# HumaticsLAB/SEAM-Match-RCNN

Measured on AMD Instinct MI355X. Metric: video-clips/sec (10f x 800^2, 32 ROI/f, 1k gallery), higher is better.
Workload: dtype f32; 1 GPU; configs[1] full pipeline, fixed ROIs: 10 frames 800x800 -> ResNet-50-FPN + RPN head -> RoIAlign 14x14 (32 ROI/frame) -> mask head -> match trunk x2 -> SEAM NLB + attention pool (32 seq x 10) -> pair logits vs 1000-product bank -> top-20; hip_graph=False, hip_streams=2, frames=10, rois_per_frame=32, gallery=1000, topk=20, parallelism=single GPU

## Files before the change

include/seam_hip.h:

```cpp
#ifndef SEAM_HIP_H
#define SEAM_HIP_H

#include <stdint.h>

#ifdef __cplusplus
extern "C" {
#endif

typedef void* seam_stream_t;

int seam_version(void);
int seam_fastdiv_exact(unsigned d, unsigned long long n_max);
const char* seam_error_string(int code);

int seam_option_count(void);
const char* seam_option_name(int index);
int seam_set_option(const char* name, int value);
int seam_get_option(const char* name, int* value);

int seam_conv_kred(int C, int R, int S);
int seam_conv_rows_padded(int K);
int seam_conv_tile(int M, int K);
int seam_conv_tile_prec(int prec, int M, int K);
int seam_conv_tile_taps(int prec, int M, int K, int taps);
// ... 185 lines not shown

int seam_paste_masks_f32(const float* masks, const float* boxes, float* out, int K, int H, int W,
                         seam_stream_t stream);

int seam_mask_select_f32(const float* logits, const int64_t* labels, float* prob, int K, int ncls,
                         seam_stream_t stream);

int seam_mask_select_f16(const void* logits, const int64_t* labels, float* prob, int K, int ncls,
                         seam_stream_t stream);

int seam_pack_conv_weight_bx3(const float* w, void* w_packed, float* tmp, int K, int Cin, int R, int S,
                              int Cstore, int mode, seam_stream_t stream);
int seam_conv2d_bx3(const float* x, const void* w_packed, const float* scale, const float* shift,
                    const float* residual, float* y, int N, int H, int W, int C, int K, int R, int S,
                    int stride, int pad, int relu, seam_stream_t stream);

int seam_wino_supported(int C, int K, int R, int S, int stride);
long long seam_wino_weight_floats(int K, int Cstore);
int seam_wino_slot_fill_pct(int N, int H, int W, int C, int K, int pad);
int seam_wino_tile_variant(int N, int H, int W, int C, int K, int pad);
int seam_pack_conv_weight_wino_f32(const float* w, float* u_packed, int K, int Cin, int Cstore, int mode,
                                   seam_stream_t stream);
int seam_conv3x3_wino_f32(const float* x, const float* u_packed, const float* scale, const float* shift,
                          const float* residual, float* y, int N, int H, int W, int C, int K, int pad, int relu,
                          seam_stream_t stream);

int seam_linear_narrow_supported(int C, int K);
int seam_pack_linear_narrow_f32(const float* w, float* w_packed, int K, int C, seam_stream_t stream);
int seam_linear_narrow_f32(const float* x, const float* w_packed, const float* bias, float* y, long long M, int C, int K,
                           int relu, seam_stream_t stream);
// ... 117 lines not shown
```

seam-match-rcnn_amd/_native.py:

```python
from __future__ import annotations

import ctypes as C
import os

import torch

_HERE = os.path.dirname(os.path.abspath(__file__))
LIB_PATH = os.environ.get("SEAM_LIB_PATH") or os.path.join(_HERE, "lib", "libseam_hip.so")

_p = C.c_void_p
_i = C.c_int
_f = C.c_float
_i64 = C.c_int64

class TrunkLayer(C.Structure):
    _fields_ = [("w", C.c_void_p), ("u", C.c_void_p), ("u24", C.c_void_p), ("scale", C.c_void_p), ("shift", C.c_void_p)]


SIGNATURES = {
    "seam_version": (_i, []),
    "seam_fastdiv_exact": (_i, [C.c_uint, C.c_ulonglong]),
    "seam_error_string": (C.c_char_p, [_i]),
    "seam_option_count": (_i, []),
    "seam_option_name": (C.c_char_p, [_i]),
# ... 20 lines not shown
    "seam_pack_conv1x1_pc_f32": (_i, [_p, _p, _i, _i, _p]),
    "seam_conv1x1_pc_f32": (_i, [_p, _p, _p, _p, _p, _p, C.c_longlong, _i, _i, _i, _p]),
    "seam_conv1x1_sw_config": (_i, [_i, _i, _i, _i]),
    "seam_conv1x1_sw_f32": (_i, [_p, _p, _p, _p, _p, _p, _i, _i, _i, _i, _i, _i, _i, _i, _i, _i, _p]),
    "seam_conv1x1_swh_config": (_i, [C.c_longlong, _i, _i, _i]),
    "seam_conv1x1_f16pc_supported": (_i, [C.c_longlong, _i, _i]),
    "seam_conv1x1_f16pc_weight_halves": (C.c_longlong, [_i, _i]),
    "seam_pack_conv1x1_weight_f16pc": (_i, [_p, _p, _i, _i, _p]),
    "seam_conv1x1_f16pc": (_i, [_p, _p, _p, _p, _p, _p, C.c_longlong, _i, _i, _i, _p]),
    "seam_conv1x1_swh_f16": (_i, [_p, _p, _p, _p, _p, _p, _p, C.c_longlong, _i, _i, _i, _i, _i, _i, _i, _i, _i, _p]),
    "seam_stem_s2d_swh_f16": (_i, [_p, _p, _p, _p, _p, _i, _i, _i, _i, _p]),
    "seam_conv2d_dual_f16": (_i, [_p, _p, _p, _p, _p, _p, _i, _i, _i, _i, _i, _i, _i, _i, _i, _i, _p]),
    "seam_conv2d_upres_f32": (_i, [_p, _p, _p, _p, _p, _p, _i, _i, _i, _i, _i, _i, _i, _i, _i, _i, _i, _i, _p]),
    "seam_pack_conv_weight_bx3": (_i, [_p, _p, _p, _i, _i, _i, _i, _i, _i, _p]),
    "seam_conv2d_bx3": (_i, [_p, _p, _p, _p, _p, _p, _i, _i, _i, _i, _i, _i, _i, _i, _i, _i, _p]),
    "seam_wino_supported": (_i, [_i, _i, _i, _i, _i]),
    "seam_wino_weight_floats": (C.c_longlong, [_i, _i]),
    "seam_wino_slot_fill_pct": (_i, [_i, _i, _i, _i, _i, _i]),
    "seam_wino_tile_variant": (_i, [_i, _i, _i, _i, _i, _i]),
    "seam_pack_conv_weight_wino_f32": (_i, [_p, _p, _i, _i, _i, _i, _p]),
    "seam_wino_issue_slots": (C.c_longlong, [_i, _i, _i, _i, _i, _i]),
    "seam_wino24_issue_slots": (C.c_longlong, [_i, _i, _i, _i, _i, _i]),
    "seam_wino24_variant": (_i, [_i, _i, _i, _i, _i, _i]),
    "seam_wino24_form": (_i, [_i, _i, _i, _i, _i, _i]),
    "seam_wino24_weight_floats": (C.c_longlong, [_i, _i]),
    "seam_pack_conv_weight_wino24_f32": (_i, [_p, _p, _i, _i, _i, _i, _p]),
    "seam_conv3x3_wino24_f32": (_i, [_p, _p, _p, _p, _p, _p, _i, _i, _i, _i, _i, _i, _i, _p]),
    "seam_conv3x3_wino_f32": (_i, [_p, _p, _p, _p, _p, _p, _i, _i, _i, _i, _i, _i, _i, _p]),
    "seam_conv3x3_f16pc_supported": (_i, [_i, _i, _i, _i, _i, _i]),
    "seam_conv3x3_f16pc_pays": (_i, [_i, _i, _i, _i, _i, _i]),
# ... 153 lines not shown
```

seam-match-rcnn_amd/csrc/seam_conv.hip:

```cpp
#include <hip/hip_runtime.h>
#include <stdint.h>
#include <stdio.h>
#include <stdlib.h>
#include "seam_fastdiv.h"
#include "seam_fpn_common.h"
#include "seam_opts.h"

typedef float f32x4 __attribute__((ext_vector_type(4)));
typedef float f32x16 __attribute__((ext_vector_type(16)));
typedef _Float16 f16x8 __attribute__((ext_vector_type(8)));
typedef unsigned u32x4 __attribute__((ext_vector_type(4)));

namespace {

constexpr int CHUNK_BYTES = 128;
constexpr int LDB = CHUNK_BYTES + 16;
constexpr unsigned kOob = 0x80000000u;

struct ConvArgs {
    const void* x;
    const void* w;
    const float* scale;
    const float* shift;
    const void* res;
// ... 716 lines not shown
#pragma unroll
                for (int r = 0; r < 16; ++r)
                    rv[r] = __builtin_bit_cast(float, __builtin_amdgcn_raw_buffer_load_b32(r_rsrc, nok ? eo[r] * 4u : kOob, 0, 0));
            }
#pragma unroll
            for (int r = 0; r < 16; ++r) {
                float v = acc[i][j][r] * sc + sh;
                if (p.res) v = p.relu == 2 ? (rv[r] > 0.f ? v : 0.f) : v + rv[r];
                if (p.relu == 1) v = fmaxf(v, 0.f);
                __builtin_amdgcn_raw_buffer_store_b32(__builtin_bit_cast(unsigned, v), y_rsrc, nok ? eo[r] * 4u : kOob, 0, 0);
            }
        }
    }
}

__global__ void split_weight_kernel(const float* __restrict__ in, unsigned short* __restrict__ out, size_t total) {
    for (size_t i = (size_t)blockIdx.x * blockDim.x + threadIdx.x; i < total; i += (size_t)gridDim.x * blockDim.x) {
        const float x = in[i];
        const __bf16 h = (__bf16)x;
        const __bf16 l = (__bf16)(x - (float)h);
        const size_t rowchunk = i >> 5;
        const int col = (int)(i & 31);
        out[rowchunk * 64 + col] = __builtin_bit_cast(unsigned short, h);
        out[rowchunk * 64 + 32 + col] = __builtin_bit_cast(unsigned short, l);
    }
}

template <typename T>
__global__ void pack_weight_kernel(const float* __restrict__ w, T* __restrict__ out, int K, int Cin, int R, int S,
                                   int Cstore, int kred, int rows, int bn, int mode) {
// ... 46 lines not shown

template <typename T>
int pack_weight(const float* w, void* w_packed, int K, int Cin, int R, int S, int Cstore, int mode, void* stream) {
    constexpr int BKE = CHUNK_BYTES / (int)sizeof(T), EPV = 16 / (int)sizeof(T);
    if ((Cstore % EPV) || (Cstore >= BKE && Cstore % BKE)) return (int)hipErrorInvalidValue;
    const int kred = kred_of<T>(Cstore, R, S);
    const int rows = ((K + 63) / 64) * 64;
    const size_t total = (size_t)rows * kred;
    int grid = (int)((total + 255) / 256);
    if (grid > 4096) grid = 4096;
    hipLaunchKernelGGL(pack_weight_kernel<T>, dim3(grid), dim3(256), 0, (hipStream_t)stream, w, (T*)w_packed, K, Cin, R, S,
                       Cstore, kred, rows, rows % 128 == 0 ? 128 : 64, mode);
    return (int)hipGetLastError();
}

enum Prec { P_F32 = 0, P_F16 = 1, P_BX3 = 2 };

inline int tile_weight(int prec, int bm, int bn, int taps) {
    const int area = bm * bn;
    if (prec == P_F32) return area == 256 * 128 ? 100 : area == 128 * 128 ? 100 : area == 64 * 64 ? 125 : 110;
    if (prec == P_F16 && area == 256 * 128) return taps >= 9 ? 92 : 105;
    return area == 256 * 128 ? 95 : area == 128 * 128 ? 100 : area == 64 * 64 ? 200 : 150;
}

inline void choose_tile(int prec, int M, int K, int& best_bm, int& best_bn, int taps = 1) {
    const int rows = ((K + 63) / 64) * 64;
    const int slab = rows % 128 == 0 ? 128 : 64;
    const int force = seam_opt::get(seam_opt::CONV_TILE);
    if (force) {
        const int fm = force / 1000, fn = force % 1000;
        if ((fm == 256 || fm == 128 || fm == 64) && (fn == 128 || fn == 64) &&
            fn <= slab && (fm != 256 || fn == 128)) {
            best_bm = fm; best_bn = fn;
            return;
        }
    }
    long best_cost = -1;
    best_bm = 128;
    best_bn = slab;
    for (int bm = 256; bm >= 64; bm >>= 1)
        for (int bn = slab; bn >= 64; bn -= 64) {
            if (bm == 256 && (bn != 128 || prec == P_F32)) continue;
            const long nb = (long)((M + bm - 1) / bm) * (rows / bn);
            const long cost = ((nb + 255) / 256) * bm * bn * tile_weight(prec, bm, bn, taps);
            if (best_cost < 0 || cost < best_cost) { best_cost = cost; best_bm = bm; best_bn = bn; }
        }
}

struct DualSrc { const void* x2; int H2, W2, C2, stride2; };

inline void set_row_split(ConvArgs& a) {
    const unsigned long long howo = (unsigned long long)a.Ho * a.Wo;
    a.m_HoWo = seam_fastdiv::magic(howo);
    a.m_Wo = seam_fastdiv::magic((unsigned long long)a.Wo);
    a.div_fast = (a.Ho > 0 && a.Wo > 0 && (howo >= 256 || seam_fastdiv::exact(howo, howo + 256)) &&
                  seam_fastdiv::exact((unsigned long long)a.Wo, howo)) ? 1 : 0;
}
// ... 59 lines not shown
            else if (best_bm == 128) hipLaunchKernelGGL((conv_igemm<T, 128, 64, 4, true>), grid, dim3(256), dyn, st, a);
            else if (best_bn == 128) hipLaunchKernelGGL((conv_igemm<T, 64, 128, 4, true>), grid, dim3(256), dyn, st, a);
            else hipLaunchKernelGGL((conv_igemm<T, 64, 64, 4, true>), grid, dim3(256), dyn, st, a);
            return (int)hipGetLastError();
        }
    }
    if (best_bm == 256) hipLaunchKernelGGL((conv_igemm<T, 256, 128, 8>), grid, dim3(512), dyn, st, a);
    else if (best_bm == 128 && best_bn == 128) hipLaunchKernelGGL((conv_igemm<T, 128, 128, 4>), grid, dim3(256), dyn, st, a);
    else if (best_bm == 128) hipLaunchKernelGGL((conv_igemm<T, 128, 64, 4>), grid, dim3(256), dyn, st, a);
    else if (best_bn == 128) hipLaunchKernelGGL((conv_igemm<T, 64, 128, 4>), grid, dim3(256), dyn, st, a);
    else hipLaunchKernelGGL((conv_igemm<T, 64, 64, 4>), grid, dim3(256), dyn, st, a);
    return (int)hipGetLastError();
}

int conv2d_bx3(const void* x, const void* w_packed, const float* scale, const float* shift, const void* residual, void* y,
               int N, int H, int W, int C, int K, int R, int S, int stride, int pad, int relu, void* stream) {
    if ((C % 4) || (C >= 32 && C % 32) || N <= 0 || K <= 0) return (int)hipErrorInvalidValue;
    ConvArgs a;
    a.x = x; a.w = w_packed; a.scale = scale; a.shift = shift; a.res = residual; a.y = y;
    a.N = N; a.H = H; a.W = W; a.C = C;
    a.Ho = (H + 2 * pad - R) / stride + 1;
    a.Wo = (W + 2 * pad - S) / stride + 1;
    a.K = K; a.R = R; a.S = S; a.stride = stride; a.pad = pad;
    a.kred = kred_of<float>(C, R, S);
    a.M = N * a.Ho * a.Wo;
    a.relu = relu;
    a.y_f32 = 1;
    a.vec_epi = 0;
    a.epi_prio = 0;
    a.rH = 0; a.rW = 0;
    a.x2 = nullptr; a.H2 = a.W2 = a.C2 = a.stride2 = 0;
    set_row_split(a);
    if (a.Ho <= 0 || a.Wo <= 0) return (int)hipErrorInvalidValue;
    const int rows = ((K + 63) / 64) * 64;
    a.slab_bn = rows % 128 == 0 ? 128 : 64;
    int best_bm, best_bn;
    choose_tile(P_BX3, a.M, K, best_bm, best_bn);
    a.tiles_m = (a.M + best_bm - 1) / best_bm;
    a.tiles_n = rows / best_bn;
    const dim3 grid(a.tiles_m * a.tiles_n);
    hipStream_t st = (hipStream_t)stream;
    if (best_bm == 256) hipLaunchKernelGGL((conv_igemm_bx3<256, 128, 8>), grid, dim3(512), 0, st, a);
    else if (best_bm == 128 && best_bn == 128) hipLaunchKernelGGL((conv_igemm_bx3<128, 128, 4>), grid, dim3(256), 0, st, a);
    else if (best_bm == 128) hipLaunchKernelGGL((conv_igemm_bx3<128, 64, 4>), grid, dim3(256), 0, st, a);
    else if (best_bn == 128) hipLaunchKernelGGL((conv_igemm_bx3<64, 128, 4>), grid, dim3(256), 0, st, a);
    else hipLaunchKernelGGL((conv_igemm_bx3<64, 64, 4>), grid, dim3(256), 0, st, a);
    return (int)hipGetLastError();
}

}

extern "C" {

int seam_conv_kred(int C, int R, int S) { return kred_of<float>(C, R, S); }
int seam_conv_kred_f16(int C, int R, int S) { return kred_of<_Float16>(C, R, S); }
int seam_conv_rows_padded(int K) { return ((K + 63) / 64) * 64; }
// ... 71 lines not shown
                              void* stream) {
    const int rc = pack_weight<float>(w, tmp, K, Cin, R, S, Cstore, mode, stream);
    if (rc) return rc;
    const size_t total = (size_t)(((K + 63) / 64) * 64) * kred_of<float>(Cstore, R, S);
    int grid = (int)((total + 255) / 256);
    if (grid > 4096) grid = 4096;
    hipLaunchKernelGGL(split_weight_kernel, dim3(grid), dim3(256), 0, (hipStream_t)stream, tmp, (unsigned short*)w_packed, total);
    return (int)hipGetLastError();
}

int seam_conv2d_bx3(const float* x, const void* w_packed, const float* scale, const float* shift, const float* residual,
                    float* y, int N, int H, int W, int C, int K, int R, int S, int stride, int pad, int relu, void* stream) {
    return conv2d_bx3(x, w_packed, scale, shift, residual, y, N, H, W, C, K, R, S, stride, pad, relu, stream);
}

}
```

seam-match-rcnn_amd/models/detection.py:

```python
from __future__ import annotations

import math
from collections import OrderedDict
from typing import List, Sequence, Tuple

import numpy as np
import torch
import torch.nn.functional as F
from torch import nn

from .. import ops

RESNET50_LAYERS = ((3, 64, 1), (4, 128, 2), (6, 256, 2), (3, 512, 2))
BBOX_XFORM_CLIP = math.log(1000.0 / 16)
NMS_MAX_BOXES = 16384


def _key(params, dtype=None) -> tuple:
    return tuple((p.data_ptr(), p._version) for p in params) + (dtype,)


def cdt(module):
    return getattr(module, "compute_dtype", torch.float32)


def adt(module) -> torch.dtype:
    return torch.float16 if cdt(module) == torch.float16 else torch.float32


def set_compute_dtype(model: nn.Module, dtype) -> nn.Module:
    if dtype not in (torch.float32, torch.float16, ops.BX3):
        raise ValueError('compute dtype must be torch.float32, torch.float16 or "bf16x3"')
    for m in model.modules():
        m.compute_dtype = dtype
    return model


def resized_size(h: int, w: int, min_size: int = 800, max_size: int = 1333) -> Tuple[int, int, float]:
    scale = min(float(min_size) / float(min(h, w)), float(max_size) / float(max(h, w)))
    return int(math.floor(float(h) * scale)), int(math.floor(float(w) * scale)), scale


# ... 25 lines not shown
        super().__init__()
        self.eps = eps
        self.register_buffer("weight", torch.ones(n))
        self.register_buffer("bias", torch.zeros(n))
        self.register_buffer("running_mean", torch.zeros(n))
        self.register_buffer("running_var", torch.ones(n))

    def _load_from_state_dict(self, state_dict, prefix, *a, **k):
        state_dict.pop(prefix + "num_batches_tracked", None)
        super()._load_from_state_dict(state_dict, prefix, *a, **k)

    def tensors(self):
        return (self.weight, self.bias, self.running_mean, self.running_var)


import os as _os
FUSE_SHORTCUT = _os.environ.get("SEAM_FUSE_SHORTCUT", "1") != "0"
STEM_S2D = _os.environ.get("SEAM_STEM_S2D", "1") != "0"
STEM_SWH = _os.environ.get("SEAM_STEM_SWH", "1") != "0"
BODY_STREAMS = int(_os.environ.get("SEAM_BODY_STREAMS", "2"))


class Bottleneck(nn.Module):
    def __init__(self, inplanes, planes, stride, downsample):
        super().__init__()
        self.conv1 = nn.Conv2d(inplanes, planes, 1, bias=False)
        self.bn1 = FrozenBatchNorm2d(planes)
        self.conv2 = nn.Conv2d(planes, planes, 3, stride, 1, bias=False)
        self.bn2 = FrozenBatchNorm2d(planes)
        self.conv3 = nn.Conv2d(planes, planes * 4, 1, bias=False)
        self.bn3 = FrozenBatchNorm2d(planes * 4)
# ... 11 lines not shown
        self.bn1 = FrozenBatchNorm2d(64)
        inpl = 64
        for li, (nblk, planes, stride) in enumerate(RESNET50_LAYERS, start=1):
            blocks = []
            for bi in range(nblk):
                blocks.append(Bottleneck(inpl, planes, stride if bi == 0 else 1, bi == 0))
                inpl = planes * 4
            setattr(self, f"layer{li}", nn.Sequential(*blocks))
        self._pk, self._pk_key = None, None

    def _all(self):
        return list(self.parameters()) + list(self.buffers())

    def packed(self):
        dt = cdt(self)
        key = _key(self._all(), dt)
        if self._pk is None or key != self._pk_key:
            with torch.no_grad():
                pk = {"stem": ops.pack_conv(self.conv1.weight, None, self.bn1.tensors(), stride=2, pad=3,
                                            cstore=8 if dt == torch.float16 else 4, bn_eps=self.bn1.eps, dtype=dt)}
                if dt in (torch.float32, torch.float16):
                    w8 = F.pad(self.conv1.weight.detach().to(torch.float32), (1, 0, 1, 0))
                    ws = w8.view(64, 3, 4, 2, 4, 2).permute(0, 3, 5, 1, 2, 4).reshape(64, 12, 4, 4).contiguous()
                    pk["stem_s2d"] = ops.pack_conv(ws, None, self.bn1.tensors(), stride=1, pad=2, cstore=12 if dt == torch.float32 else 16,
                                                   bn_eps=self.bn1.eps, wino=False, dtype=dt)
                    if dt == torch.float16 and STEM_SWH:
                        pk["stem_rows"] = F.pad(ws, (0, 0, 0, 0, 0, 4)).permute(0, 2, 3, 1).reshape(64, 256).to(torch.float16).contiguous()
                for li in range(1, 5):
                    for bi, b in enumerate(getattr(self, f"layer{li}")):
                        e = {"c1": ops.pack_conv(b.conv1.weight, None, b.bn1.tensors(), bn_eps=b.bn1.eps, dtype=dt),
                             "c2": ops.pack_conv(b.conv2.weight, None, b.bn2.tensors(), stride=b.stride, pad=1,
                                                 bn_eps=b.bn2.eps, dtype=dt),
                             "c3": ops.pack_conv(b.conv3.weight, None, b.bn3.tensors(), bn_eps=b.bn3.eps, dtype=dt)}
                        if b.downsample is not None:
                            e["ds"] = ops.pack_conv(b.downsample[0].weight, None, b.downsample[1].tensors(),
                                                    stride=b.stride, bn_eps=b.downsample[1].eps, dtype=dt)
                            if dt in (torch.float32, torch.float16) and FUSE_SHORTCUT:
                                e["c3ds"] = ops.pack_conv_dual(b.conv3.weight, b.bn3.tensors(), b.downsample[0].weight,
                                                               b.downsample[1].tensors(), bn_eps=b.bn3.eps, dtype=dt)
                        pk[(li, bi)] = e
            self._pk, self._pk_key = pk, key
        return self._pk

    def forward(self, x: torch.Tensor, s2d_padded: bool = False, taped: bool = False) -> List[torch.Tensor]:
        if taped:
            return self.forward_taped(x, s2d_padded)
        pk = self.packed()
        n = x.shape[0]
        if BODY_STREAMS >= 2 and n >= 2 * BODY_STREAMS and x.is_cuda:
            cur = torch.cuda.current_stream()
            if (getattr(self, "_streams", None) is None or len(self._streams) != BODY_STREAMS
                    or self._streams[0].device != x.device):
                self._streams = [torch.cuda.Stream(device=x.device) for _ in range(BODY_STREAMS)]
            spad = 3 if s2d_padded else 0
# ... 20 lines not shown
        if x.shape[-1] in (12, 16):
            streaming = ("stem_rows" in pk and x.dtype == torch.float16 and x.shape[-1] == 16
                         and (x.shape[1] - (3 if s2d_padded else 0)) * (x.shape[2] - (3 if s2d_padded else 0)) >= 128)
            if s2d_padded and not streaming:
                x = x[:, 2:-1, 2:-1].contiguous()
            if streaming:
                x = ops.stem_s2d_f16(x, pk["stem_rows"], pk["stem_s2d"].scale, pk["stem_s2d"].shift, relu=True, padded=s2d_padded)
            else:
                x = ops.conv2d(x, pk["stem_s2d"], relu=True, out_hw=(x.shape[1], x.shape[2]))
        else:
            x = ops.conv2d(x, pk["stem"], relu=True)
        return ops.maxpool2d(x, 3, 2, 1)

    def _run(self, x, pk, outs, s2d_padded=False):
        x = self._stem(x, pk, s2d_padded)
        feats = []
        for li in range(1, 5):
            nblk = len(getattr(self, f"layer{li}"))
            for bi in range(nblk):
                e = pk[(li, bi)]
                o = ops.conv2d(x, e["c1"], relu=True)
                o = ops.conv2d(o, e["c2"], relu=True)
                if "c3ds" in e:
                    x = ops.conv2d_dual(o, x, e["c3ds"], getattr(self, f"layer{li}")[bi].stride, relu=True)
                    continue
                idt = ops.conv2d(x, e["ds"]) if "ds" in e else x
                x = ops.conv2d(o, e["c3"], relu=True, residual=idt,
                               out=outs[li - 1] if (outs is not None and bi == nblk - 1) else None)
            feats.append(x)
        return feats

    def blocks(self):
        return [(li, bi, b) for li in range(1, 5) for bi, b in enumerate(getattr(self, f"layer{li}"))]

    def forward_taped(self, x: torch.Tensor, s2d_padded: bool = False) -> List[torch.Tensor]:
        from ..autograd import BodyFunction
        if cdt(self) != torch.float32 or x.dtype != torch.float32:
            raise NotImplementedError("the training branch of the ResNet body is fp32 only: call set_compute_dtype(torch.float32)")
        if self.conv1.weight.requires_grad:
            raise NotImplementedError(
                "ResNet body training: the stem of the backbone (backbone.body.conv1 and its max-pool) has no backward; freeze "
                "it with `model.backbone.body.conv1.weight.requires_grad_(False)` or build the model with "
# ... 544 lines not shown
```

seam-match-rcnn_amd/ops.py:

```python
from __future__ import annotations

import ctypes as C
from dataclasses import dataclass
from typing import Optional, Sequence

import torch

from . import _native

F32 = torch.float32
F16 = torch.float16


def _stream() -> int:
    return torch.cuda.current_stream().cuda_stream


def _req(t: torch.Tensor, dtype=F32, name: str = "tensor") -> torch.Tensor:
    if not isinstance(t, torch.Tensor) or not t.is_cuda:
        raise _native.SeamNativeError(f"{name}: expected a tensor on the HIP device (no CPU path exists)")
    if dtype is not None and t.dtype != dtype:
        raise TypeError(f"{name}: expected {dtype}, got {t.dtype}")
    return t if t.is_contiguous() else t.contiguous()

# ... 22 lines not shown
    pad: int = 0
    Cin: int = 0
    dtype: object = F32
    u: Optional[torch.Tensor] = None
    u24: Optional[torch.Tensor] = None
    wn: Optional[torch.Tensor] = None
    ws: Optional[torch.Tensor] = None
    shift_sw: Optional[torch.Tensor] = None
    wq: Optional[torch.Tensor] = None
    wh: Optional[torch.Tensor] = None
    wsh: Optional[torch.Tensor] = None
    wph: Optional[torch.Tensor] = None


BX3 = "bf16x3"


import os as _os
WINOGRAD = _os.environ.get("SEAM_WINOGRAD", "1") != "0"
F16PC = _os.environ.get("SEAM_F16PC", "1") != "0"
F16PC64 = _os.environ.get("SEAM_F16PC64", "1") != "0"
PWPC = _os.environ.get("SEAM_PWPC", "1") != "0"
SWH = _os.environ.get("SEAM_PWH", "1") != "0"
PWHPC = _os.environ.get("SEAM_PWHPC", "1") != "0"
PWHPC_MIN_C = int(_os.environ.get("SEAM_PWHPC_MIN_C", "1024"))
F16PC_RULE = True


def _pack_wino(lib, weight: torch.Tensor, K: int, cin: int, cs: int, mode: int) -> Optional[torch.Tensor]:
    if not lib.seam_wino_supported(cs, K, 3, 3, 1):
# ... 95 lines not shown
    u = u24 = wh = None
    if dtype == F32:
        kred = lib.seam_conv_kred(cs, R, S)
        wp = torch.empty((rows, kred), dtype=F32, device=weight.device)
        _native.check(lib.seam_pack_conv_weight_f32(_ptr(weight), _ptr(wp), K, cin, R, S, cs, mode, _stream()),
                      "seam_pack_conv_weight_f32")
        if wino and mode == 0 and R == 3 and S == 3 and stride == 1:
            u = _pack_wino(lib, weight, K, cin, cs, 0)
            u24 = _pack_wino24(lib, weight, K, cin, cs, 0) if u is not None else None
    elif dtype == BX3:
        kred = lib.seam_conv_kred(cs, R, S)
        wp = torch.empty((rows, kred), dtype=F32, device=weight.device)
        tmp = torch.empty((rows, kred), dtype=F32, device=weight.device)
        _native.check(lib.seam_pack_conv_weight_bx3(_ptr(weight), _ptr(wp), _ptr(tmp), K, cin, R, S, cs, mode, _stream()),
                      "seam_pack_conv_weight_bx3")
    else:
        kred = lib.seam_conv_kred_f16(cs, R, S)
        wp = torch.empty((rows, kred), dtype=F16, device=weight.device)
        _native.check(lib.seam_pack_conv_weight_f16(_ptr(weight), _ptr(wp), K, cin, R, S, cs, mode, _stream()),
                      "seam_pack_conv_weight_f16")
        if F16PC and mode == 0 and R == 3 and S == 3 and stride == 1 and pad in (0, 1) and ((cs % 128 == 0 and K % 128 == 0) or (cs == 64 and K == 64 and F16PC64)):
            wh = torch.empty((int(lib.seam_f16pc_weight_halves(K, cs)),), dtype=F16, device=weight.device)
            _native.check(lib.seam_pack_conv_weight_f16pc(_ptr(weight), _ptr(wh), K, cin, cs, _stream()), "seam_pack_conv_weight_f16pc")
    scale = shift = None
    if bias is not None:
        bias = bias.detach().to(F32)
        if transposed2x2:
            bias = bias.repeat(4)
    if bn is not None:
        bw, bb, rm, rv = (t.detach().to(F32) for t in bn)
# ... 248 lines not shown
                                              n * h * w, c, pc.K, int(relu), _stream()), "seam_conv1x1_pc_f32")
    elif wino24:
        _native.check(lib.seam_conv3x3_wino24_f32(_ptr(x), _ptr(pc.u24), _ptr(pc.scale), _ptr(pc.shift), _ptr(residual), _ptr(y),
                                                  n, h, w, c, pc.K, pc.pad, int(relu), _stream()), "seam_conv3x3_wino24_f32")
    elif wino:
        _native.check(lib.seam_conv3x3_wino_f32(_ptr(x), _ptr(pc.u), _ptr(pc.scale), _ptr(pc.shift), _ptr(residual), _ptr(y),
                                                n, h, w, c, pc.K, pc.pad, int(relu), _stream()), "seam_conv3x3_wino_f32")
    elif out_hw is not None:
        crop = lib.seam_conv2d_crop_f16 if pc.dtype == F16 else lib.seam_conv2d_crop_f32
        _native.check(crop(_ptr(x), _ptr(pc.w), _ptr(pc.scale), _ptr(pc.shift), _ptr(y), n, h, w, c, pc.K,
                           pc.R, pc.S, pc.stride, pc.pad, ho, wo, int(relu), _stream()), "seam_conv2d_crop")
    elif pc.dtype == F32:
        _native.check(lib.seam_conv2d_f32(_ptr(x), _ptr(pc.w), _ptr(pc.scale), _ptr(pc.shift), _ptr(residual), _ptr(y),
                                          n, h, w, c, pc.K, pc.R, pc.S, pc.stride, pc.pad, int(relu), _stream()),
                      "seam_conv2d_f32")
    elif pc.dtype == BX3:
        _native.check(lib.seam_conv2d_bx3(_ptr(x), _ptr(pc.w), _ptr(pc.scale), _ptr(pc.shift), _ptr(residual), _ptr(y),
                                          n, h, w, c, pc.K, pc.R, pc.S, pc.stride, pc.pad, int(relu), _stream()),
                      "seam_conv2d_bx3")
    elif f16pc:
        _native.check(lib.seam_conv3x3_f16pc(_ptr(x), _ptr(pc.wh), _ptr(pc.scale), _ptr(pc.shift), None, _ptr(y),
                                             n, h, w, c, pc.K, pc.pad, 1 if relu else 0, _stream()), "seam_conv3x3_f16pc")
    else:
        _native.check(lib.seam_conv2d_f16(_ptr(x), _ptr(pc.w), _ptr(pc.scale), _ptr(pc.shift), _ptr(residual), _ptr(y),
                                          n, h, w, c, pc.K, pc.R, pc.S, pc.stride, pc.pad, 1 if relu else 0,
                                          1 if out_f32 else 0, _stream()), "seam_conv2d_f16")
    if trace is not None:
        e1.record()
        tile = lib.seam_conv_tile_taps(2 if pc.dtype == BX3 else 1 if pc.dtype == F16 else 0, n * ho * wo, pc.K, pc.R * pc.S)
        if pwhpc:
            variant = "conv1x1_f16pc"
        elif swh:
            variant = _swh_variant(lib, n * h * w, c, pc.K)
        elif narrow:
            variant = "linear_narrow"
        elif sw:
            variant = _sw_variant(lib, n * h * w, c, pc.K)
        elif pwpc:
            variant = "conv1x1_pc"
        elif wino24:
            variant = ("conv3x3_wino24pc" if lib.seam_wino24_form(n, h, w, c, pc.K, pc.pad) == 1
                       else f"conv3x3_wino24<{lib.seam_wino24_variant(n, h, w, c, pc.K, pc.pad)}>")
        elif wino:
            variant = f"conv3x3_wino<{lib.seam_wino_tile_variant(n, h, w, c, pc.K, pc.pad)}>"
        elif f16pc:
            variant = "conv3x3_f16pc"
        elif pc.dtype == BX3:
            variant = f"conv_igemm_bx3<{tile // 1000},{tile % 1000}>"
        else:
            variant = f"conv_igemm<{'float' if pc.dtype == F32 else '_Float16'},{tile // 1000},{tile % 1000}>"
        es = x.element_size()
        trace.append((variant, 2.0 * n * ho * wo * pc.K * pc.R * pc.S * (pc.Cin or pc.Cstore), e0, e1,
                      (n, h, w, c, pc.K, pc.R, pc.stride),
                      float(es * (x.numel() + pc.w.numel()) + y.element_size() * y.numel()
                            + (es * y.numel() if residual is not None else 0))))
    return y


def stem_s2d_f16(x: torch.Tensor, w_rows: torch.Tensor, scale: Optional[torch.Tensor], shift: Optional[torch.Tensor],
                 relu: bool = True, padded: bool = False) -> torch.Tensor:
    x = _req(x, F16, "x")
# ... 920 lines not shown
```

Before: 72.41 clips/s.

## Add bf16x6/x9 split-precision MFMA conv path for f32 backbone bottleneck convs

Adds a new implicit-GEMM conv kernel that splits f32 activations and weights into three bf16 pieces each and accumulates six or nine bf16 MFMA cross products, emulating f32 accuracy on matrix cores. The backbone's 1x1 reduce, stride-2 3x3 and wide 1x1 expand convolutions use this path by default when running f32 inference. It aims to replace slower f32 SIMT or bf16x3 conv kernels with matrix-core throughput, at the cost of more MFMA issues per tile, extra LDS for three operand planes, and a small accuracy loss when six terms are used.

```diff
diff --git a/include/seam_hip.h b/include/seam_hip.h
--- a/include/seam_hip.h
+++ b/include/seam_hip.h
@@ -223,6 +223,12 @@
 int seam_conv2d_bx3(const float* x, const void* w_packed, const float* scale, const float* shift,
                     const float* residual, float* y, int N, int H, int W, int C, int K, int R, int S,
                     int stride, int pad, int relu, seam_stream_t stream);
+
+int seam_pack_conv_weight_sx(const float* w, void* w_packed, float* tmp, int K, int Cin, int R, int S,
+                             int Cstore, int mode, seam_stream_t stream);
+int seam_conv2d_sx(const float* x, const void* w_packed, const float* scale, const float* shift,
+                   const float* residual, float* y, int N, int H, int W, int C, int K, int R, int S,
+                   int stride, int pad, int relu, int terms, seam_stream_t stream);
 
 int seam_wino_supported(int C, int K, int R, int S, int stride);
 long long seam_wino_weight_floats(int K, int Cstore);
diff --git a/seam-match-rcnn_amd/_native.py b/seam-match-rcnn_amd/_native.py
--- a/seam-match-rcnn_amd/_native.py
+++ b/seam-match-rcnn_amd/_native.py
@@ -58,6 +58,8 @@
     "seam_conv2d_upres_f32": (_i, [_p, _p, _p, _p, _p, _p, _i, _i, _i, _i, _i, _i, _i, _i, _i, _i, _i, _i, _p]),
     "seam_pack_conv_weight_bx3": (_i, [_p, _p, _p, _i, _i, _i, _i, _i, _i, _p]),
     "seam_conv2d_bx3": (_i, [_p, _p, _p, _p, _p, _p, _i, _i, _i, _i, _i, _i, _i, _i, _i, _i, _p]),
+    "seam_pack_conv_weight_sx": (_i, [_p, _p, _p, _i, _i, _i, _i, _i, _i, _p]),
+    "seam_conv2d_sx": (_i, [_p, _p, _p, _p, _p, _p, _i, _i, _i, _i, _i, _i, _i, _i, _i, _i, _i, _p]),
     "seam_wino_supported": (_i, [_i, _i, _i, _i, _i]),
     "seam_wino_weight_floats": (C.c_longlong, [_i, _i]),
     "seam_wino_slot_fill_pct": (_i, [_i, _i, _i, _i, _i, _i]),
diff --git a/seam-match-rcnn_amd/csrc/seam_conv.hip b/seam-match-rcnn_amd/csrc/seam_conv.hip
--- a/seam-match-rcnn_amd/csrc/seam_conv.hip
+++ b/seam-match-rcnn_amd/csrc/seam_conv.hip
@@ -754,6 +754,349 @@
     }
 }
 
+__device__ __forceinline__ float top16(float x) {
+    unsigned t = __builtin_bit_cast(unsigned, x) & 0xffff0000u;
+    asm volatile("" : "+v"(t));
+    return __builtin_bit_cast(float, t);
+}
+
+__device__ __forceinline__ void split3_bf16(const f32x4 v, u32x2& p0, u32x2& p1, u32x2& p2) {
+#pragma unroll
+    for (int p = 0; p < 2; ++p) {
+        const float a0 = top16(v[2 * p]), b0 = top16(v[2 * p + 1]);
+        const float ra = v[2 * p] - a0, rb = v[2 * p + 1] - b0;
+        const float a1 = top16(ra), b1 = top16(rb);
+        const float sa = ra - a1, sb = rb - b1;
+        p0[p] = (__builtin_bit_cast(unsigned, a0) >> 16) | __builtin_bit_cast(unsigned, b0);
+        p1[p] = (__builtin_bit_cast(unsigned, a1) >> 16) | __builtin_bit_cast(unsigned, b1);
+        p2[p] = (__builtin_bit_cast(unsigned, sa) >> 16) | (__builtin_bit_cast(unsigned, sb) & 0xffff0000u);
+    }
+}
+
+template <int BM, int BN, int TERMS>
+__global__ __launch_bounds__(256, BM * BN >= 128 * 128 ? 1 : 2) void conv_igemm_sx(const ConvArgs p) {
+    static_assert(TERMS == 6 || TERMS == 9, "six or nine piece products");
+    constexpr int NW = 4, ES = 4, EPV = 4, BKE = 32;
+    constexpr int WM = BM / 2, WN = BN / 2;
+    constexpr int MT = WM / 32, NT = WN / 32;
+    constexpr int RP = 8 * NW;
+    constexpr int AI = BM / RP;
+    constexpr int VPP = BN * 4;
+    constexpr int BI = 3 * VPP / 256;
+    constexpr int Q = TERMS * MT * NT;
+    constexpr int PA = BM * 64 + 64;
+    constexpr int PB = BN * 64 + 64;
+
+    __shared__ __attribute__((aligned(16))) char As[2][3 * PA];
+    __shared__ __attribute__((aligned(16))) char Bs[2][3 * PB];
+
+    const int tid = threadIdx.x;
+    const int lane = tid & 63;
+    const int wid = tid >> 6;
+    const int wm0 = (wid >> 1) * WM;
+    const int wn0 = (wid & 1) * WN;
+
+    const int nblk = gridDim.x;
+    const int b = blockIdx.x;
+    const int xcd = b & 7;
+    const int q8 = nblk >> 3, rem = nblk & 7;
+    const int tile = (xcd < rem ? xcd * (q8 + 1) : rem * (q8 + 1) + (xcd - rem) * q8) + (b >> 3);
+    const int tm = tile / p.tiles_n;
+    const int tn = tile - tm * p.tiles_n;
+    const int m0 = tm * BM;
+    const int n0 = tn * BN;
+
+    const int nk = p.kred / BKE;
+    const int lcol = tid & 7;
+    const int lrow = tid >> 3;
+    const int HoWo = p.Ho * p.Wo;
+    const int n_first = m0 / HoWo;
+    const size_t img_elems = (size_t)p.H * p.W * p.C;
+    const size_t rem_bytes = ((size_t)(p.N - n_first) * img_elems) * ES;
+    const __amdgpu_buffer_rsrc_t a_rsrc = __builtin_amdgcn_make_buffer_rsrc(
+        (void*)((const char*)p.x + (size_t)n_first * img_elems * ES), 0,
+        (int)(rem_bytes > kOob ? kOob : (unsigned)rem_bytes), 0x00020000);
+    const int slab_stride = p.slab_bn * 192;
+    const int n_in_slab = n0 % p.slab_bn;
+    const __amdgpu_buffer_rsrc_t b_rsrc = __builtin_amdgcn_make_buffer_rsrc(
+        (void*)((const char*)p.w + (size_t)(n0 - n_in_slab) * p.kred * 6), 0,
+        (int)((unsigned)nk * (unsigned)slab_stride), 0x00020000);
+
+    int arow[AI], ahi[AI], awi[AI];
+#pragma unroll
+    for (int i = 0; i < AI; ++i) {
+        const int m = m0 + lrow + RP * i;
+        if (m < p.M) {
+            const int n = m / HoWo;
+            const int rm = m - n * HoWo;
+            const int ho = rm / p.Wo;
+            const int wo = rm - ho * p.Wo;
+            ahi[i] = ho * p.stride - p.pad;
+            awi[i] = wo * p.stride - p.pad;
+            arow[i] = ((((n - n_first) * p.H + ahi[i]) * p.W + awi[i]) * p.C) * ES;
+        } else {
+            ahi[i] = -(1 << 28);
+            awi[i] = 0;
+            arow[i] = 0;
+        }
+    }
+    int brow[BI];
+#pragma unroll
+    for (int i = 0; i < BI; ++i) {
+        const int pl = (256 * i) / VPP, within = tid + (256 * i) % VPP;
+        brow[i] = pl * p.slab_bn * 64 + (n_in_slab + (within >> 2)) * 64 + (within & 3) * 16;
+    }
+
+    int kc, kr, ks, tapoff;
+    {
+        const int kk = lcol * EPV;
+        const int pos = kk / p.C;
+        kc = kk - pos * p.C;
+        kr = pos / p.S;
+        ks = pos - kr * p.S;
+        tapoff = ((kr * p.W + ks) * p.C + kc) * ES;
+    }
+    int uq = 0;
+
+    constexpr int D = 2;
+    f32x4 areg[D][AI], breg[D][BI];
+    auto load_a = [&](f32x4 (&ar)[AI], int i) {
+        const bool ok = (unsigned)(ahi[i] + kr) < (unsigned)p.H && (unsigned)(awi[i] + ks) < (unsigned)p.W && kr < p.R;
+        const unsigned off = ok ? (unsigned)(arow[i] + tapoff) : kOob;
+        if (!(SEAM_BX3_ABL & 1)) ar[i] = __builtin_bit_cast(f32x4, __builtin_amdgcn_raw_buffer_load_b128(a_rsrc, off, 0, 0));
+    };
+    auto load_b = [&](f32x4 (&br)[BI], int i) {
+        const int so = uq < nk ? uq * slab_stride : (int)kOob;
+        if (!(SEAM_BX3_ABL & 1)) br[i] = __builtin_bit_cast(f32x4, __builtin_amdgcn_raw_buffer_load_b128(b_rsrc, brow[i], so, 0));
+    };
+    auto advance_k = [&]() {
+        ++uq;
+        if (p.C >= BKE) {
+            if (++ks == p.S) {
+                ks = 0;
+                kc += BKE;
+                if (kc >= p.C) { kc -= p.C; ++kr; }
+            }
+        } else {
+            kc += BKE;
+            while (kc >= p.C) {
+                kc -= p.C;
+                if (++ks == p.S) { ks = 0; ++kr; }
+            }
+        }
+        tapoff = ((kr * p.W + ks) * p.C + kc) * ES;
+    };
+    auto load_chunk = [&](f32x4 (&ar)[AI], f32x4 (&br)[BI]) {
+#pragma unroll
+        for (int i = 0; i < AI; ++i) load_a(ar, i);
+#pragma unroll
+        for (int i = 0; i < BI; ++i) load_b(br, i);
+        advance_k();
+    };
+    auto store_row = [&](const f32x4 (&ar)[AI], const f32x4 (&br)[BI], int buf, int r) {
+        if (SEAM_BX3_ABL & 2) return;
+        if (r < AI) {
+            const int row = lrow + RP * r;
+            const int off = row * 64 + ((((lcol >> 1) ^ (row >> 2)) & 3) << 4) + (lcol & 1) * 8;
+            u32x2 q0, q1, q2;
+            if (SEAM_BX3_ABL & 4) { q0[0] = __builtin_bit_cast(unsigned, ar[r][0]); q0[1] = __builtin_bit_cast(unsigned, ar[r][1]);
+                                    q1[0] = __builtin_bit_cast(unsigned, ar[r][2]); q1[1] = __builtin_bit_cast(unsigned, ar[r][3]); q2 = q0; }
+            else split3_bf16(ar[r], q0, q1, q2);
+            *reinterpret_cast<u32x2*>(&As[buf][off]) = q0;
+            *reinterpret_cast<u32x2*>(&As[buf][PA + off]) = q1;
+            *reinterpret_cast<u32x2*>(&As[buf][2 * PA + off]) = q2;
+        } else {
+            const int i = r - AI;
+            const int pl = (256 * i) / VPP, within = tid + (256 * i) % VPP;
+            const int row = within >> 2;
+            *reinterpret_cast<f32x4*>(&Bs[buf][pl * PB + row * 64 + ((((within & 3) ^ (row >> 2)) & 3) << 4)]) = br[i];
+        }
+    };
+
+    f32x16 acc[MT][NT];
+#pragma unroll
+    for (int i = 0; i < MT; ++i)
+#pragma unroll
+        for (int j = 0; j < NT; ++j)
+#pragma unroll
+            for (int r = 0; r < 16; ++r) acc[i][j][r] = 0.f;
+
+    const int arow0 = wm0 + (lane & 31), brow0 = wn0 + (lane & 31);
+    struct Frag { f32x4 a[3][MT], b[3][NT]; };
+    Frag f0, f1;
+    auto read_frags = [&](Frag& f, int buf, int step) {
+        if (SEAM_BX3_ABL & 16) return;
+        const int slot = 2 * step + (lane >> 5);
+#pragma unroll
+        for (int i = 0; i < MT; ++i) {
+            const int row = arow0 + i * 32;
+            const int off = row * 64 + (((slot ^ (row >> 2)) & 3) << 4);
+#pragma unroll
+            for (int pl = 0; pl < 3; ++pl) f.a[pl][i] = *reinterpret_cast<const f32x4*>(&As[buf][pl * PA + off]);
+        }
+#pragma unroll
+        for (int j = 0; j < NT; ++j) {
+            const int row = brow0 + j * 32;
+            const int off = row * 64 + (((slot ^ (row >> 2)) & 3) << 4);
+#pragma unroll
+            for (int pl = 0; pl < 3; ++pl) f.b[pl][j] = *reinterpret_cast<const f32x4*>(&Bs[buf][pl * PB + off]);
+        }
+    };
+    auto mf = [&](const Frag& f, int idx) {
+        constexpr int T9[9] = {2 * 4 + 2, 2 * 4 + 1, 1 * 4 + 2, 2 * 4 + 0, 1 * 4 + 1, 0 * 4 + 2, 1 * 4 + 0, 0 * 4 + 1, 0};
+        const int term = T9[idx / (MT * NT) + (9 - TERMS)], i = (idx / NT) % MT, j = idx % NT;
+        acc[i][j] = __builtin_amdgcn_mfma_f32_32x32x16_bf16(__builtin_bit_cast(bf16x8, f.a[term >> 2][i]),
+                                                            __builtin_bit_cast(bf16x8, f.b[term & 3][j]), acc[i][j], 0, 0, 0);
+    };
+
+    auto chunk = [&](int buf, f32x4 (&lda)[AI], f32x4 (&ldb)[BI], const f32x4 (&sta)[AI], const f32x4 (&stb)[BI]) {
+        read_frags(f1, buf, 1);
+#pragma unroll
+        for (int q = 0; q < Q; ++q) {
+            mf(f0, q);
+#pragma unroll
+            for (int i = 0; i < AI + BI; ++i)
+                if ((i * Q) / (AI + BI) == q) {
+                    if (i < AI) load_a(lda, i);
+                    else load_b(ldb, i - AI);
+                }
+            if (q == Q - 1) advance_k();
+        }
+        constexpr int QS = (2 * Q) / 3;
+#pragma unroll
+        for (int q = 0; q < Q; ++q) {
+            mf(f1, q);
+#pragma unroll
+            for (int r = 0; r < AI + BI; ++r)
+                if ((r * QS) / (AI + BI) == q) store_row(sta, stb, buf ^ 1, r);
+            if (q == QS - 1) {
+                if (!(SEAM_BX3_ABL & 8)) __syncthreads();
+                read_frags(f0, buf ^ 1, 0);
+            }
+        }
+    };
+
+    load_chunk(areg[0], breg[0]);
+#pragma unroll
+    for (int r = 0; r < AI + BI; ++r) store_row(areg[0], breg[0], 0, r);
+    load_chunk(areg[1], breg[1]);
+    __syncthreads();
+    read_frags(f0, 0, 0);
+
+    for (int t = 0; t < nk; t += 2) {
+        chunk(0, areg[0], breg[0], areg[1], breg[1]);
+        if (t + 1 < nk) chunk(1, areg[1], breg[1], areg[0], breg[0]);
+    }
+    __syncthreads();
+
+    const size_t tile_off = (size_t)m0 * p.K;
+    const unsigned rows_here = (unsigned)min(BM, p.M - m0);
+    const __amdgpu_buffer_rsrc_t y_rsrc = __builtin_amdgcn_make_buffer_rsrc(
+        (void*)((char*)p.y + tile_off * 4), 0, (int)(rows_here * (unsigned)p.K * 4), 0x00020000);
+    const __amdgpu_buffer_rsrc_t r_rsrc = __builtin_amdgcn_make_buffer_rsrc(
+        (void*)((const char*)(p.res ? p.res : p.y) + tile_off * 4), 0, (int)(rows_here * (unsigned)p.K * 4), 0x00020000);
+    if ((p.K & 3) == 0) {
+        constexpr int EW = WN + 4;
+        constexpr int LPR = WN / 4;
+        constexpr int RPI = 64 / LPR;
+        constexpr int NP = 32 / RPI;
+        static_assert(4 * 32 * EW * 4 <= 2 * 3 * (BM >= BN ? PA : PB), "the transpose fits the operand's LDS");
+        float* eb = reinterpret_cast<float*>(BM >= BN ? &As[0][0] : &Bs[0][0]) + wid * 32 * EW;
+        const int er = lane / LPR, ec = (lane % LPR) * 4;
+        const int n = n0 + wn0 + ec;
+        const bool nok = n < p.K;
+        f32x4 sc = {1.f, 1.f, 1.f, 1.f}, sh = {0.f, 0.f, 0.f, 0.f};
+        if (p.scale && nok) sc = *reinterpret_cast<const f32x4*>(p.scale + n);
+        if (p.shift && nok) sh = *reinterpret_cast<const f32x4*>(p.shift + n);
+#pragma unroll
+        for (int i = 0; i < MT; ++i) {
+            unsigned eo[NP];
+            f32x4 rv[NP];
+#pragma unroll
+            for (int k = 0; k < NP; ++k) {
+                const int row = wm0 + i * 32 + k * RPI + er;
+                eo[k] = nok ? (unsigned)(row * p.K + n) * 4u : kOob;
+            }
+            if (p.res) {
+#pragma unroll
+                for (int k = 0; k < NP; ++k)
+                    rv[k] = __builtin_bit_cast(f32x4, __builtin_amdgcn_raw_buffer_load_b128(r_rsrc, eo[k], 0, 0));
+                __builtin_amdgcn_sched_barrier(0);
+            }
+#pragma unroll
+            for (int j = 0; j < NT; ++j)
+#pragma unroll
+                for (int r = 0; r < 16; ++r)
+                    eb[((r & 3) + 8 * (r >> 2) + 4 * (lane >> 5)) * EW + j * 32 + (lane & 31)] = acc[i][j][r];
+#pragma unroll
+            for (int k = 0; k < NP; ++k) {
+                f32x4 v = *reinterpret_cast<const f32x4*>(&eb[(k * RPI + er) * EW + ec]) * sc + sh;
+                if (p.res) {
+                    if (p.relu == 2) {
+#pragma unroll
+                        for (int e = 0; e < 4; ++e) v[e] = rv[k][e] > 0.f ? v[e] : 0.f;
+                    } else {
+                        v += rv[k];
+                    }
+                }
+                if (p.relu == 1) {
+#pragma unroll
+                    for (int e = 0; e < 4; ++e) v[e] = fmaxf(v[e], 0.f);
+                }
+                __builtin_amdgcn_raw_buffer_store_b128(__builtin_bit_cast(u32x4, v), y_rsrc, eo[k], 0, 0);
+            }
+        }
+        return;
+    }
+#pragma unroll
+    for (int j = 0; j < NT; ++j) {
+        const int n = n0 + wn0 + j * 32 + (lane & 31);
+        const bool nok = n < p.K;
+        const float sc = (p.scale && nok) ? p.scale[n] : 1.f;
+        const float sh = (p.shift && nok) ? p.shift[n] : 0.f;
+#pragma unroll
+        for (int i = 0; i < MT; ++i) {
+            unsigned eo[16];
+            float rv[16];
+#pragma unroll
+            for (int r = 0; r < 16; ++r) {
+                const int row = wm0 + i * 32 + (r & 3) + 8 * (r >> 2) + 4 * (lane >> 5);
+                eo[r] = (unsigned)(row * p.K + n);
+            }
+            if (p.res) {
+#pragma unroll
+                for (int r = 0; r < 16; ++r)
+                    rv[r] = __builtin_bit_cast(float, __builtin_amdgcn_raw_buffer_load_b32(r_rsrc, nok ? eo[r] * 4u : kOob, 0, 0));
+            }
+#pragma unroll
+            for (int r = 0; r < 16; ++r) {
+                float v = acc[i][j][r] * sc + sh;
+                if (p.res) v = p.relu == 2 ? (rv[r] > 0.f ? v : 0.f) : v + rv[r];
+                if (p.relu == 1) v = fmaxf(v, 0.f);
+                __builtin_amdgcn_raw_buffer_store_b32(__builtin_bit_cast(unsigned, v), y_rsrc, nok ? eo[r] * 4u : kOob, 0, 0);
+            }
+        }
+    }
+}
+
+__global__ void split3_weight_kernel(const float* __restrict__ in, unsigned short* __restrict__ out, size_t total, int slab_bn) {
+    for (size_t i = (size_t)blockIdx.x * blockDim.x + threadIdx.x; i < total; i += (size_t)gridDim.x * blockDim.x) {
+        const float x = in[i];
+        const unsigned x0 = __builtin_bit_cast(unsigned, x) & 0xffff0000u;
+        const float r = x - __builtin_bit_cast(float, x0);
+        const unsigned y0 = __builtin_bit_cast(unsigned, r) & 0xffff0000u;
+        const float s = r - __builtin_bit_cast(float, y0);
+        const size_t rowchunk = i >> 5;
+        const int col = (int)(i & 31);
+        const size_t slabchunk = rowchunk / (size_t)slab_bn;
+        const int row = (int)(rowchunk - slabchunk * slab_bn);
+        unsigned short* o = out + slabchunk * 3 * (size_t)slab_bn * 32 + (size_t)row * 32 + col;
+        o[0] = (unsigned short)(x0 >> 16);
+        o[(size_t)slab_bn * 32] = (unsigned short)(y0 >> 16);
+        o[(size_t)slab_bn * 64] = (unsigned short)(__builtin_bit_cast(unsigned, s) >> 16);
+    }
+}
+
 __global__ void split_weight_kernel(const float* __restrict__ in, unsigned short* __restrict__ out, size_t total) {
     for (size_t i = (size_t)blockIdx.x * blockDim.x + threadIdx.x; i < total; i += (size_t)gridDim.x * blockDim.x) {
         const float x = in[i];
@@ -830,12 +1173,13 @@
     return (int)hipGetLastError();
 }
 
-enum Prec { P_F32 = 0, P_F16 = 1, P_BX3 = 2 };
+enum Prec { P_F32 = 0, P_F16 = 1, P_BX3 = 2, P_SX = 3 };
 
 inline int tile_weight(int prec, int bm, int bn, int taps) {
     const int area = bm * bn;
     if (prec == P_F32) return area == 256 * 128 ? 100 : area == 128 * 128 ? 100 : area == 64 * 64 ? 125 : 110;
     if (prec == P_F16 && area == 256 * 128) return taps >= 9 ? 92 : 105;
+    if (prec == P_SX) return area == 128 * 128 ? 117 : area == 64 * 64 ? 110 : bm == 64 ? 100 : 106;
     return area == 256 * 128 ? 95 : area == 128 * 128 ? 100 : area == 64 * 64 ? 200 : 150;
 }
 
@@ -846,7 +1190,7 @@
     if (force) {
         const int fm = force / 1000, fn = force % 1000;
         if ((fm == 256 || fm == 128 || fm == 64) && (fn == 128 || fn == 64) &&
-            fn <= slab && (fm != 256 || fn == 128)) {
+            fn <= slab && (fm != 256 || (fn == 128 && prec != P_SX))) {
             best_bm = fm; best_bn = fn;
             return;
         }
@@ -856,7 +1200,7 @@
     best_bn = slab;
     for (int bm = 256; bm >= 64; bm >>= 1)
         for (int bn = slab; bn >= 64; bn -= 64) {
-            if (bm == 256 && (bn != 128 || prec == P_F32)) continue;
+            if (bm == 256 && (bn != 128 || prec == P_F32 || prec == P_SX)) continue;
             const long nb = (long)((M + bm - 1) / bm) * (rows / bn);
             const long cost = ((nb + 255) / 256) * bm * bn * tile_weight(prec, bm, bn, taps);
             if (best_cost < 0 || cost < best_cost) { best_cost = cost; best_bm = bm; best_bn = bn; }
@@ -946,7 +1290,7 @@
 }
 
 int conv2d_bx3(const void* x, const void* w_packed, const float* scale, const float* shift, const void* residual, void* y,
-               int N, int H, int W, int C, int K, int R, int S, int stride, int pad, int relu, void* stream) {
+               int N, int H, int W, int C, int K, int R, int S, int stride, int pad, int relu, void* stream, int terms = 3) {
     if ((C % 4) || (C >= 32 && C % 32) || N <= 0 || K <= 0) return (int)hipErrorInvalidValue;
     ConvArgs a;
     a.x = x; a.w = w_packed; a.scale = scale; a.shift = shift; a.res = residual; a.y = y;
@@ -967,11 +1311,25 @@
     const int rows = ((K + 63) / 64) * 64;
     a.slab_bn = rows % 128 == 0 ? 128 : 64;
     int best_bm, best_bn;
-    choose_tile(P_BX3, a.M, K, best_bm, best_bn);
+    choose_tile(terms == 3 ? P_BX3 : P_SX, a.M, K, best_bm, best_bn);
     a.tiles_m = (a.M + best_bm - 1) / best_bm;
     a.tiles_n = rows / best_bn;
     const dim3 grid(a.tiles_m * a.tiles_n);
     hipStream_t st = (hipStream_t)stream;
+    if (terms != 3) {
+        if (terms != 6 && terms != 9) return (int)hipErrorInvalidValue;
+#define SEAM_SX_LAUNCH(BM_, BN_)                                                                          \
+        do {                                                                                              \
+            if (terms == 6) hipLaunchKernelGGL((conv_igemm_sx<BM_, BN_, 6>), grid, dim3(256), 0, st, a);  \
+            else hipLaunchKernelGGL((conv_igemm_sx<BM_, BN_, 9>), grid, dim3(256), 0, st, a);             \
+        } while (0)
+        if (best_bm == 128 && best_bn == 128) SEAM_SX_LAUNCH(128, 128);
+        else if (best_bm == 128) SEAM_SX_LAUNCH(128, 64);
+        else if (best_bn == 128) SEAM_SX_LAUNCH(64, 128);
+        else SEAM_SX_LAUNCH(64, 64);
+#undef SEAM_SX_LAUNCH
+        return (int)hipGetLastError();
+    }
     if (best_bm == 256) hipLaunchKernelGGL((conv_igemm_bx3<256, 128, 8>), grid, dim3(512), 0, st, a);
     else if (best_bm == 128 && best_bn == 128) hipLaunchKernelGGL((conv_igemm_bx3<128, 128, 4>), grid, dim3(256), 0, st, a);
     else if (best_bm == 128) hipLaunchKernelGGL((conv_igemm_bx3<128, 64, 4>), grid, dim3(256), 0, st, a);
@@ -1073,4 +1431,24 @@
     return conv2d_bx3(x, w_packed, scale, shift, residual, y, N, H, W, C, K, R, S, stride, pad, relu, stream);
 }
 
-}
+int seam_pack_conv_weight_sx(const float* w, void* w_packed, float* tmp, int K, int Cin, int R, int S, int Cstore, int mode,
+                             void* stream) {
+    const int rc = pack_weight<float>(w, tmp, K, Cin, R, S, Cstore, mode, stream);
+    if (rc) return rc;
+    const int rows = ((K + 63) / 64) * 64;
+    const size_t total = (size_t)rows * kred_of<float>(Cstore, R, S);
+    int grid = (int)((total + 255) / 256);
+    if (grid > 4096) grid = 4096;
+    hipLaunchKernelGGL(split3_weight_kernel, dim3(grid), dim3(256), 0, (hipStream_t)stream, tmp, (unsigned short*)w_packed, total,
+                       rows % 128 == 0 ? 128 : 64);
+    return (int)hipGetLastError();
+}
+
+int seam_conv2d_sx(const float* x, const void* w_packed, const float* scale, const float* shift, const float* residual,
+                   float* y, int N, int H, int W, int C, int K, int R, int S, int stride, int pad, int relu, int terms,
+                   void* stream) {
+    if (terms != 6 && terms != 9) return (int)hipErrorInvalidValue;
+    return conv2d_bx3(x, w_packed, scale, shift, residual, y, N, H, W, C, K, R, S, stride, pad, relu, stream, terms);
+}
+
+}
diff --git a/seam-match-rcnn_amd/models/detection.py b/seam-match-rcnn_amd/models/detection.py
--- a/seam-match-rcnn_amd/models/detection.py
+++ b/seam-match-rcnn_amd/models/detection.py
@@ -16,6 +16,9 @@
 NMS_MAX_BOXES = 16384
 
 
+import os as _os
+
+
 def _key(params, dtype=None) -> tuple:
     return tuple((p.data_ptr(), p._version) for p in params) + (dtype,)
 
@@ -26,6 +29,23 @@
 
 def adt(module) -> torch.dtype:
     return torch.float16 if cdt(module) == torch.float16 else torch.float32
+
+
+SPLIT_F32 = _os.environ.get("SEAM_SPLIT_F32", "1") != "0"
+SPLIT_DTYPE = {"6": ops.SX6, "9": ops.SX9}[_os.environ.get("SEAM_SPLIT_TERMS", "6")]
+SPLIT_C3_MIN_C = 256
+SPLIT_CLASSES = frozenset(c for c in _os.environ.get("SEAM_SPLIT_CLASSES", "c1,c3,c2s2").split(",") if c)
+
+
+def split_on(module) -> bool:
+    return (SPLIT_F32 and getattr(module, "split_f32", True) and cdt(module) == torch.float32 and not module.training
+            and not torch.is_grad_enabled())
+
+
+def set_split_f32(model: nn.Module, on: bool) -> nn.Module:
+    for m in model.modules():
+        m.split_f32 = bool(on)
+    return model
 
 
 def set_compute_dtype(model: nn.Module, dtype) -> nn.Module:
@@ -81,7 +101,6 @@
         return (self.weight, self.bias, self.running_mean, self.running_var)
 
 
-import os as _os
 FUSE_SHORTCUT = _os.environ.get("SEAM_FUSE_SHORTCUT", "1") != "0"
 STEM_S2D = _os.environ.get("SEAM_STEM_S2D", "1") != "0"
 STEM_SWH = _os.environ.get("SEAM_STEM_SWH", "1") != "0"
@@ -123,7 +142,8 @@
 
     def packed(self):
         dt = cdt(self)
-        key = _key(self._all(), dt)
+        sx = dt == torch.float32 and SPLIT_F32 and getattr(self, "split_f32", True)
+        key = _key(self._all(), dt) + (sx,)
         if self._pk is None or key != self._pk_key:
             with torch.no_grad():
                 pk = {"stem": ops.pack_conv(self.conv1.weight, None, self.bn1.tensors(), stride=2, pad=3,
@@ -147,6 +167,14 @@
                             if dt in (torch.float32, torch.float16) and FUSE_SHORTCUT:
                                 e["c3ds"] = ops.pack_conv_dual(b.conv3.weight, b.bn3.tensors(), b.downsample[0].weight,
                                                                b.downsample[1].tensors(), bn_eps=b.bn3.eps, dtype=dt)
+                        if sx:
+                            if "c1" in SPLIT_CLASSES:
+                                e["c1x"] = ops.pack_conv(b.conv1.weight, None, b.bn1.tensors(), bn_eps=b.bn1.eps, dtype=SPLIT_DTYPE)
+                            if "c2s2" in SPLIT_CLASSES and b.stride == 2:
+                                e["c2x"] = ops.pack_conv(b.conv2.weight, None, b.bn2.tensors(), stride=2, pad=1, bn_eps=b.bn2.eps,
+                                                         dtype=SPLIT_DTYPE)
+                            if "c3" in SPLIT_CLASSES and "c3ds" not in e and b.conv3.in_channels >= SPLIT_C3_MIN_C:
+                                e["c3x"] = ops.pack_conv(b.conv3.weight, None, b.bn3.tensors(), bn_eps=b.bn3.eps, dtype=SPLIT_DTYPE)
                         pk[(li, bi)] = e
             self._pk, self._pk_key = pk, key
         return self._pk
@@ -197,18 +225,19 @@
 
     def _run(self, x, pk, outs, s2d_padded=False):
         x = self._stem(x, pk, s2d_padded)
+        sx = split_on(self)
         feats = []
         for li in range(1, 5):
             nblk = len(getattr(self, f"layer{li}"))
             for bi in range(nblk):
                 e = pk[(li, bi)]
-                o = ops.conv2d(x, e["c1"], relu=True)
-                o = ops.conv2d(o, e["c2"], relu=True)
+                o = ops.conv2d(x, e.get("c1x", e["c1"]) if sx else e["c1"], relu=True)
+                o = ops.conv2d(o, e.get("c2x", e["c2"]) if sx else e["c2"], relu=True)
                 if "c3ds" in e:
                     x = ops.conv2d_dual(o, x, e["c3ds"], getattr(self, f"layer{li}")[bi].stride, relu=True)
                     continue
                 idt = ops.conv2d(x, e["ds"]) if "ds" in e else x
-                x = ops.conv2d(o, e["c3"], relu=True, residual=idt,
+                x = ops.conv2d(o, e.get("c3x", e["c3"]) if sx else e["c3"], relu=True, residual=idt,
                                out=outs[li - 1] if (outs is not None and bi == nblk - 1) else None)
             feats.append(x)
         return feats
diff --git a/seam-match-rcnn_amd/ops.py b/seam-match-rcnn_amd/ops.py
--- a/seam-match-rcnn_amd/ops.py
+++ b/seam-match-rcnn_amd/ops.py
@@ -60,6 +60,9 @@
 
 
 BX3 = "bf16x3"
+SX6 = "bf16x6"
+SX9 = "bf16x9"
+_SX_TERMS = {SX6: 6, SX9: 9}
 
 
 import os as _os
@@ -185,6 +188,12 @@
         tmp = torch.empty((rows, kred), dtype=F32, device=weight.device)
         _native.check(lib.seam_pack_conv_weight_bx3(_ptr(weight), _ptr(wp), _ptr(tmp), K, cin, R, S, cs, mode, _stream()),
                       "seam_pack_conv_weight_bx3")
+    elif dtype in _SX_TERMS:
+        kred = lib.seam_conv_kred(cs, R, S)
+        wp = torch.empty((rows, kred * 3), dtype=torch.bfloat16, device=weight.device)
+        tmp = torch.empty((rows, kred), dtype=F32, device=weight.device)
+        _native.check(lib.seam_pack_conv_weight_sx(_ptr(weight), _ptr(wp), _ptr(tmp), K, cin, R, S, cs, mode, _stream()),
+                      "seam_pack_conv_weight_sx")
     else:
         kred = lib.seam_conv_kred_f16(cs, R, S)
         wp = torch.empty((rows, kred), dtype=F16, device=weight.device)
@@ -463,6 +472,10 @@
         _native.check(lib.seam_conv2d_f32(_ptr(x), _ptr(pc.w), _ptr(pc.scale), _ptr(pc.shift), _ptr(residual), _ptr(y),
                                           n, h, w, c, pc.K, pc.R, pc.S, pc.stride, pc.pad, int(relu), _stream()),
                       "seam_conv2d_f32")
+    elif pc.dtype in _SX_TERMS:
+        _native.check(lib.seam_conv2d_sx(_ptr(x), _ptr(pc.w), _ptr(pc.scale), _ptr(pc.shift), _ptr(residual), _ptr(y),
+                                         n, h, w, c, pc.K, pc.R, pc.S, pc.stride, pc.pad, int(relu), _SX_TERMS[pc.dtype], _stream()),
+                      "seam_conv2d_sx")
     elif pc.dtype == BX3:
         _native.check(lib.seam_conv2d_bx3(_ptr(x), _ptr(pc.w), _ptr(pc.scale), _ptr(pc.shift), _ptr(residual), _ptr(y),
                                           n, h, w, c, pc.K, pc.R, pc.S, pc.stride, pc.pad, int(relu), _stream()),
@@ -476,7 +489,8 @@
                                           1 if out_f32 else 0, _stream()), "seam_conv2d_f16")
     if trace is not None:
         e1.record()
-        tile = lib.seam_conv_tile_taps(2 if pc.dtype == BX3 else 1 if pc.dtype == F16 else 0, n * ho * wo, pc.K, pc.R * pc.S)
+        tile = lib.seam_conv_tile_taps(3 if pc.dtype in _SX_TERMS else 2 if pc.dtype == BX3 else 1 if pc.dtype == F16 else 0,
+                                       n * ho * wo, pc.K, pc.R * pc.S)
         if pwhpc:
             variant = "conv1x1_f16pc"
         elif swh:
@@ -494,6 +508,8 @@
             variant = f"conv3x3_wino<{lib.seam_wino_tile_variant(n, h, w, c, pc.K, pc.pad)}>"
         elif f16pc:
             variant = "conv3x3_f16pc"
+        elif pc.dtype in _SX_TERMS:
+            variant = f"conv_igemm_sx<{tile // 1000},{tile % 1000},{_SX_TERMS[pc.dtype]}>"
         elif pc.dtype == BX3:
             variant = f"conv_igemm_bx3<{tile // 1000},{tile % 1000}>"
         else:
```

Result: faster. 73.69 clips/s (median of 6 runs) (+1.8%).
